# 959AI994/Multi-Gate-VAE

Measured on AMD Instinct MI355X. Metric: circuit-graphs/sec (train step), AIG-64k batch=64 per GPU, higher is better.
Workload: dtype f32 storage; dense products as bf16x3 split-precision MFMA, fp32 accumulate; 1 GPU; cfg2: DG_AE --type aig, 64 x 65536-node synthetic levelised DAGs per GPU (N=4194304, E=6558720, 120 levels), H=64, 4+4 rounds, layernorm, weights [1,4,4], negatives sampled; step includes the 7-scalar metrics copy (pinned, read one step behind); global_batch=64, parallelism=dp1

## Files before the change

### include/mgvae_hip.h

```cpp
#ifndef MGVAE_HIP_H
#define MGVAE_HIP_H
#include <stdint.h>
#ifdef __cplusplus
extern "C" {
#endif

#ifndef MGV_OK
#define MGV_OK 0
#define MGV_EINVAL (-1)
#define MGV_EUNSUPPORTED (-2)
#endif

int mgv_abi_version(void);

int mgv_struct_stage_fwd(int H, int64_t N, const float* h_in, const int32_t* nbr_ptr, const int32_t* nbr_idx,
                         const uint8_t* xcls, const float* xtab, int C, const float* Wc, const float* bc,
                         const float* Whh, const float* bhh, const float* ln_w, const float* ln_b, float ln_eps,
                         float* h_out, void* stream);
int mgv_struct_stage_bwd(int H, int64_t N, const float* h_in, const int32_t* nbr_ptr, const int32_t* nbr_idx,
                         const uint8_t* xcls, const float* xtab, int C, const float* Wc, const float* WcT,
                         const float* bc, const float* Whh, const float* WhhT, const float* bhh,
                         const float* ln_w, const float* ln_b, float ln_eps, const float* gy_direct,
                         const float* gy_agg, float* g_direct_out, float* g_agg_out, float* dWc, float* dbc,
                         float* dWhh, float* dbhh, float* dxtab, float* dln_w, float* dln_b, void* stream);
int mgv_struct_stage_rows_fwd(int H, int64_t N, const float* h_in, const int32_t* nbr_ptr, const int32_t* nbr_idx,
                              const float* xrow, const float* Wc, const float* bc, const float* Whh, const float* bhh,
                              const float* ln_w, const float* ln_b, float ln_eps, float* h_out, void* stream);
int mgv_struct_stage_rows_bwd(int H, int64_t N, const float* h_in, const int32_t* nbr_ptr, const int32_t* nbr_idx,
                              const float* xrow, const float* Wc, const float* WcT, const float* bc, const float* Whh,
                              const float* WhhT, const float* bhh, const float* ln_w, const float* ln_b, float ln_eps,
                              const float* gy_direct, const float* gy_agg, float* g_direct_out, float* g_agg_out,
                              float* dWc, float* dbc, float* dWhh, float* dbhh, float* d_xrow, float* dln_w, float* dln_b,
                              void* stream);

int mgv_struct_stage_fwd_x3(int H, int64_t N, const float* h_in, const int32_t* nbr_ptr, const int32_t* nbr_idx,
                            const uint8_t* xcls, const float* xtab, int C, const void* wpack_bf16, const float* bc,
                            const float* bhh, const float* ln_w, const float* ln_b, float ln_eps, float* h_out,
                            int heavy_n, const int32_t* heavy_nodes, float* heavy_ws, const int32_t* table_own_idx,
                            int nbr_tagged, float* ln_stats_out, void* stream);
int mgv_struct_stage_bwd_x3(int H, int64_t N, const float* h_in, const int32_t* nbr_ptr, const int32_t* nbr_idx,
                            const uint8_t* xcls, const float* xtab, int C, const void* wpack_bf16, const float* bc,
                            const float* bhh, const float* ln_w, const float* ln_b, float ln_eps,
                            const float* gy_direct, const float* gy_agg, float* g_direct_out, float* g_agg_out,
                            float* dWc, float* dbc, float* dWhh, float* dbhh, float* dxtab, float* dln_w,
                            float* dln_b, int heavy_n, const int32_t* heavy_nodes, float* heavy_ws, const int32_t* table_own_idx,
                            int nbr_tagged, void* stream);

int mgv_struct_stage_bwd2_ws_floats(int H, int64_t N);
int mgv_struct_stage_bwd2_x3(int H, int64_t N, const float* h_in, const int32_t* nbr_ptr, const int32_t* nbr_idx,
                             const uint8_t* xcls, const float* xtab, int C, const void* wpack_bf16, const float* bc,
                             const float* bhh, const float* ln_w, const float* ln_b, float ln_eps,
                             const float* gy_direct, const float* gy_agg, float* g_direct_out, float* g_agg_out,
                             float* dWc, float* dbc, float* dWhh, float* dbhh, float* dxtab, float* dln_w,
                             float* dln_b, float* workspace, int64_t workspace_floats, int heavy_n,
                             const int32_t* heavy_nodes, float* heavy_ws, const int32_t* table_own_idx,
                             int nbr_tagged, const float* ln_stats, void* stream);

int mgv_linear_fwd(int64_t N, const float* X1, int K1, int ld1, const float* X2, int K2, int ld2,
                   const float* W, const float* b, int M, float* Y, int ldy, void* stream);
int mgv_linear_wgrad(int64_t N, const float* X1, int K1, int ld1, const float* X2, int K2, int ld2,
                     const float* dY, int lddy, int M, float* dW, float* db, void* stream);
int mgv_linear_x3_supported(int M, int K);
int mgv_wpack_bf16x3(const float* W, int R, int K, int ldw, int transpose, void* hi, void* lo, void* stream);
int mgv_linear_fwd_x3(int64_t N, const float* X1, int K1, int ld1, const float* X2, int K2, int ld2,
                      const void* wpack_bf16, const float* b, int M, float* Y, int ldy, void* stream);
int mgv_grouped_linear_supported(int M, int K);
int mgv_grouped_linear_fwd_x3(int64_t ntiles, const int32_t* tile_list, const int32_t* order, const int32_t* tile_start,
                              const int32_t* tile_count, const int32_t* tile_slot, const float* X, int K, int ldx,
                              const void* wpack_bf16, const float* b, int M, const float* R, int ldr, float* Y, int ldy, void* stream);
int mgv_grouped_linear_wgrad_x3_ws_floats(int M, int K, int64_t ntiles);
int mgv_grouped_linear_wgrad_x3(int64_t ntiles, const int32_t* tile_list, const int32_t* order, const int32_t* tile_start,
                                const int32_t* tile_count, const float* X, int K, int ldx, const float* dY, int lddy, int M,
                                float* dW, float* db, float* workspace, int64_t workspace_floats, void* stream);
int mgv_linear_fwd_x3_res(int64_t N, const float* X1, int K1, int ld1, const float* X2, int K2, int ld2,
                          const void* wpack_bf16, const float* b, int M, const float* R, int ldr, float* Y, int ldy,
                          void* stream);
int mgv_linear_wgrad_x3_ws_floats(int M, int K, int64_t N);
int mgv_linear_wgrad_x3(int64_t N, const float* X1, int K1, int ld1, const float* X2, int K2, int ld2,
                        const float* dY, int lddy, int M, float* dW, float* db, float* workspace, int64_t workspace_floats,
                        void* stream);
int mgv_linear_bwd_x3_supported(int M, int K);
int mgv_linear_bwd_x3(int64_t N, const float* X1, int K1, int ld1, const float* X2, int K2, int ld2, const float* dY, int lddy,
                      int M, const void* wtpack_bf16, float* dW, float* db, float* dX1, int ldx1, float* dX2, int ldx2,
                      const float* R, int ldr, float* workspace, int64_t workspace_floats, void* stream);
int mgv_gather_sum(int H, int64_t N, const float* h, const int32_t* nbr_ptr, const int32_t* nbr_idx,
                   float* agg, float* deg, void* stream);

int mgv_class_expand(int H, int64_t N, const float* table, const int32_t* class_id, float* out, void* stream);
int mgv_seg_sum(int H, int64_t n_seg, const int32_t* seg_ptr, const int32_t* items, const float* direct, const float* agg,
// ... 276 lines not shown
```

### multi-gate-vae_amd/deepgate/_model_base.py

```python
import os

import torch
from torch import nn

from . import metrics, ops, pairs, similarity
from .arch.mlp import MLP
from .arch.tfmlp import TFMlpAggr
from .data import plan_of
from .digae_layer import DirectedInnerProductDecoder
from .sampling import NegativeEdges, negative_sampling, negative_sampling_device

EPS = 1e-15
DEVICE_SAMPLER = True
MAX_LOGSTD = 10


class FunctionalModel(nn.Module):
    ENCODER_ATTR = 'struct_encoder'
    GATES = ()

    VAR_HEADS = ('fc_s_mu', 'fc_s_logstd', 'fc_t_mu', 'fc_t_logstd')

    def __init__(self, struct_encoder, num_rounds=1, dim_hidden=128, enable_encode=True, enable_reverse=True, variational=False):
        super().__init__()
        setattr(self, self.ENCODER_ATTR, struct_encoder)
        self.decoder = DirectedInnerProductDecoder()
        self.hs_linear = nn.Linear(dim_hidden * 2, dim_hidden)
        self.hs_decompose = nn.Linear(dim_hidden, dim_hidden * 2)
        self.num_rounds = num_rounds
        self.enable_encode = enable_encode
        self.enable_reverse = enable_reverse
        self.dim_hidden = dim_hidden
        self.dim_mlp = 32
        for name, _ in self.GATES:
            setattr(self, 'aggr_%s_func' % name, TFMlpAggr(dim_hidden * 2, dim_hidden))
        for name, _ in self.GATES:
            setattr(self, 'update_%s_func' % name, nn.GRU(dim_hidden, dim_hidden))
        self.readout_prob = MLP(dim_hidden, self.dim_mlp, 1, num_layer=3, p_drop=0.2, norm_layer='batchnorm',
                                act_layer='relu')
        self.variational = bool(variational)
        if self.variational:
            for name in self.VAR_HEADS:
                setattr(self, name, nn.Linear(dim_hidden, dim_hidden))
        self._klsum, self._kl_n = None, 0
        self.last_confusion = None
        self.last_link_metrics = None
        self._neg_scope, self._neg_reverse = 'batch', 0.0

    def _sweep_params(self):
        parts = [getattr(self, 'aggr_%s_func' % n).composed(getattr(self, 'update_%s_func' % n)) for n, _ in self.GATES]
        return [torch.stack([p[i] for p in parts]) for i in range(5)]

    def forward(self, G, branch=None):
        if self.num_rounds < 1:
            raise ValueError('num_rounds must be >= 1')
        plan = plan_of(G, [gid for _, gid in self.GATES])
        dev = self.hs_linear.weight.device
        rows = torch.eye(6, dtype=torch.float32, device=dev)
        enc = getattr(self, self.ENCODER_ATTR)
        s, t = enc(None, None, G.edge_index, plan=plan, classes=(rows, plan.xcls))
        hs = ops.linear(s, self.hs_linear.weight, self.hs_linear.bias, x2=t)
        hs_in = hs
        if branch is not None:
            with branch.fork(hs):
                hs_in = branch.took(*self.recon_loss(hs, plan=plan, return_hs=True, **branch.recon_args))
        hf = ops.FuncSweepFn.apply(plan, hs_in, *self._sweep_params())
        if branch is not None:
            hf = branch.sweep_out(hf)
        for _ in range(self.num_rounds - 1):
            au, Wvc, bvc, bih, _ = self._sweep_params()
            hf = ops.FuncSweepFn.apply(plan, hs_in, au, Wvc, bvc, bih, None, hf, self._round_gh(plan, hf))
        return hs, hf

    def _round_gh(self, plan, hf):
        H = self.dim_hidden
        if hf.is_cuda and H == 64 and ops.use_x3(H) and ops.GROUPED_ROUND:
            grus = [getattr(self, 'update_%s_func' % name) for name, _ in self.GATES]
            return ops.RoundGhFn.apply(plan, hf, torch.stack([g.weight_hh_l0 for g in grus]), torch.stack([g.bias_hh_l0 for g in grus]))
        gh = torch.zeros(hf.shape[0], 3 * H, dtype=hf.dtype, device=hf.device)
        for (name, _), idx in zip(self.GATES, plan.slot_nodes()):
            if idx.numel() == 0:
                continue
            gru = getattr(self, 'update_%s_func' % name)
# ... 191 lines not shown
```

### multi-gate-vae_amd/deepgate/digae_layer.py

```python
import torch
import torch.nn as nn

from . import metrics, ops, pairs
from .arch.gcn_conv import AggConv
from .graph_plan import GraphPlan

MAX_FEATURE_CLASSES = 8


def feature_classes(x):
    rows, inv = torch.unique(x, dim=0, return_inverse=True)
    if rows.shape[0] > MAX_FEATURE_CLASSES:
        return None
    return rows.to(torch.float32), inv.to(torch.uint8).contiguous()


class DirectedInnerProductDecoder(nn.Module):

    def forward(self, s, t, edge_index, sigmoid=True):
        return ops.edge_dot(s, t, edge_index, sigmoid)

    def forward_all(self, s, t, sigmoid=True):
        return pairs.pair_scores(s, t, sigmoid)

# ... 110 lines not shown
    def forward(self, s_0, t_0, edge_index, plan=None, classes=None):
        if plan is None:
            plan = GraphPlan(edge_index, (classes[1] if classes is not None else s_0).shape[0])
        F_ = self.source_conv.conv.lin.in_features
        cs = _classes_once(s_0, classes, F_)
        ct = cs if (classes is not None or t_0 is s_0) else _classes_once(t_0, None, F_)
        return self.source_conv(t_0, edge_index, plan, ct), self.target_conv(s_0, edge_index, plan, cs)


class MultiGCNEncoder(nn.Module):
    def __init__(self, num_rounds, dim_hidden, dim_feature, enable_reverse, layernorm):
        super().__init__()
        self.num_rounds = num_rounds
        self.enable_reverse = True
        self.layernorm = layernorm
        self.dim_feature = dim_feature
        self.dim_hidden = dim_hidden
        self.aggr = AggConv(dim_hidden, dim_hidden)
        self.update = nn.GRU(dim_hidden + dim_feature, dim_hidden)
        self.aggr_r = AggConv(dim_hidden, dim_hidden)
        self.update_r = nn.GRU(dim_hidden + dim_feature, dim_hidden)
        if self.layernorm:
            self.ln = nn.LayerNorm(dim_hidden)

    def _composed(self, aggr, gru, feat_rows):
        H = self.dim_hidden
        w_ih = gru.weight_ih_l0
        w_m = w_ih[:, :H]
        Wc = w_m @ aggr.msg.weight
        bc = w_m @ aggr.msg.bias
        xtab = feat_rows @ w_ih[:, H:].t() + gru.bias_ih_l0
        return xtab, Wc, bc, gru.weight_hh_l0, gru.bias_hh_l0

    def _forward_rows(self, x, edge_index, plan):
        H, F_ = self.dim_hidden, self.dim_feature
        if plan is None:
            plan = GraphPlan(edge_index, x.shape[0])
        pad = (-F_) % 16
        xp = torch.nn.functional.pad(x.to(torch.float32), (0, pad)).contiguous()
        args = []
        for aggr, gru in ((self.aggr, self.update), (self.aggr_r, self.update_r)):
            w_ih = gru.weight_ih_l0
            w_m = w_ih[:, :H]
            w_x = torch.nn.functional.pad(w_ih[:, H:], (0, pad))
            xrow = torch.cat([ops.linear(xp, w_x[g * H:(g + 1) * H], gru.bias_ih_l0[g * H:(g + 1) * H]) for g in range(3)], dim=1)
            args += [xrow, w_m @ aggr.msg.weight, w_m @ aggr.msg.bias, gru.weight_hh_l0, gru.bias_hh_l0]
        ln_w = self.ln.weight if self.layernorm else None
        ln_b = self.ln.bias if self.layernorm else None
        return ops.StructEncoderRowsFn.apply(plan, self.num_rounds, *args, ln_w, ln_b)

    def forward(self, x, edge_index, plan=None, classes=None):
        if classes is None:
            if x.shape[1] != self.dim_feature:
                raise ValueError('expected %d node features, got %d' % (self.dim_feature, x.shape[1]))
            classes = feature_classes(x)
        if classes is None:
            return self._forward_rows(x, edge_index, plan)
        rows, xcls = classes
        if rows.shape[1] != self.dim_feature:
            raise ValueError('expected %d node features, got %d' % (self.dim_feature, rows.shape[1]))
        if plan is None:
            plan = GraphPlan(edge_index, xcls.shape[0])
        rows = rows.to(self.update.weight_ih_l0.device)
        f = self._composed(self.aggr, self.update, rows)
        r = self._composed(self.aggr_r, self.update_r, rows)
        ln_w = self.ln.weight if self.layernorm else None
        ln_b = self.ln.bias if self.layernorm else None
        return ops.StructEncoderFn.apply(plan, xcls, self.num_rounds, *f, *r, ln_w, ln_b)


class DirectMultiGCNEncoder(nn.Module):
    def __init__(self, dim_feature=3, dim_hidden=128, s_rounds=1, t_rounds=1, enable_reverse=True, layernorm=False):
        super().__init__()
        self.source_conv = MultiGCNEncoder(s_rounds, dim_hidden, dim_feature, enable_reverse, layernorm)
        self.target_conv = MultiGCNEncoder(t_rounds, dim_hidden, dim_feature, enable_reverse, layernorm)

    def forward(self, s, t, edge_index, plan=None, classes=None):
        if plan is None:
            plan = GraphPlan(edge_index, s.shape[0])
        cs = classes if classes is not None else feature_classes(s)
        ct = cs if (classes is not None or t is s) else feature_classes(t)
        return self.source_conv(s, edge_index, plan, cs), self.target_conv(t, edge_index, plan, ct)
```

### multi-gate-vae_amd/deepgate/ops.py

```python
from collections import namedtuple
import math
import os

import torch

from . import _hip
from ._hip import F32, I32, U8, HipLibraryError, check, edge_rows, ptr

LN_EPS = 1e-5

PRECISION = os.environ.get('MGV_PRECISION', 'x3')
FIRST_STAGE_TABLE = True


def use_x3(H):
    return PRECISION == 'x3' and H in (32, 64)


def split_bf16(w):
    hi = w.to(torch.bfloat16)
    lo = (w - hi.to(torch.float32)).to(torch.bfloat16)
    return hi, lo


# ... 7 lines not shown
    n = W.numel()
    if W.dtype != F32 or not W.is_cuda or W.stride(1) != 1:
        raise HipLibraryError('weight must be an fp32 GPU matrix with contiguous rows')
    base = out.data_ptr() + 2 * off
    _hip.call('mgv_wpack_bf16x3', ptr(W), R, K, W.stride(0), int(transpose), _hip.ctypes.c_void_p(base),
              _hip.ctypes.c_void_p(base + 2 * n))
    return off + 2 * n


def stage_wpack(Wc, Whh):
    out = torch.empty(4 * (Wc.numel() + Whh.numel()), dtype=torch.bfloat16, device=Wc.device)
    off = 0
    for w, tr in ((Wc, False), (Whh, False), (Wc, True), (Whh, True)):
        off = _pack_into(out, off, w, tr)
    return out


def sweep_wpack(Wvc):
    out = torch.empty(4 * Wvc.numel(), dtype=torch.bfloat16, device=Wvc.device)
    off = 0
    for g in range(Wvc.shape[0]):
        off = _pack_into(out, off, Wvc[g], False)
        off = _pack_into(out, off, Wvc[g], True)
    return out


def linear_wpack(W):
    out = torch.empty(2 * W.numel(), dtype=torch.bfloat16, device=W.device)
    _pack_into(out, 0, W, False)
    return out


def _zeros_like_params(*ts):
    return [torch.zeros_like(t) for t in ts]


def _heavy_args(heavy, H, device):
    if heavy is None or heavy[0] == 0:
        return 0, None, None
    n, nodes = heavy
    return n, ptr(nodes), ptr(workspace(2 * n * H, device, tag='heavy'))


def struct_stage_fwd(h_in, nbr_ptr, nbr_idx, xcls, xtab, Wc, bc, Whh, bhh, ln_w, ln_b, out=None, wpack=None, heavy=None, table_own=None, n_rows=None,
                     stats_out=None, tagged=True):
    N, H = h_in.shape
    if n_rows is not None:
        N = int(n_rows)
    if table_own is not None:
        N = table_own.numel()
    check(h_in, F32, 'h_in'); check(nbr_ptr, I32, 'nbr_ptr'); check(nbr_idx, I32, 'nbr_idx'); check(xcls, U8, 'xcls')
    for n, t in (('xtab', xtab), ('Wc', Wc), ('bc', bc), ('Whh', Whh), ('bhh', bhh)):
        check(t, F32, n)
    check(ln_w, F32, 'ln_w'); check(ln_b, F32, 'ln_b')
    assert nbr_ptr.numel() == N + 1 and xcls.numel() == N
    assert Wc.shape == (3 * H, H) and Whh.shape == (3 * H, H) and xtab.shape[1] == 3 * H
    h_out = (torch.empty(N, H, dtype=F32, device=h_in.device) if out is None else out)
    if use_x3(H):
        wpack = stage_wpack(Wc, Whh) if wpack is None else wpack
        _hip.call('mgv_struct_stage_fwd_x3', H, N, ptr(h_in), ptr(nbr_ptr), ptr(nbr_idx), ptr(xcls), ptr(xtab),
                  xtab.shape[0], ptr(wpack), ptr(bc), ptr(bhh), ptr(ln_w), ptr(ln_b), LN_EPS, ptr(h_out), *_heavy_args(heavy, H, h_in.device), ptr(table_own),
                  int(bool(tagged)), ptr(stats_out))
        return h_out
    assert table_own is None, 'table mode needs the bf16x3 kernels'
    _hip.call('mgv_struct_stage_fwd', H, N, ptr(h_in), ptr(nbr_ptr), ptr(nbr_idx), ptr(xcls), ptr(xtab),
              xtab.shape[0], ptr(Wc), ptr(bc), ptr(Whh), ptr(bhh), ptr(ln_w), ptr(ln_b), LN_EPS, ptr(h_out))
    return h_out
# ... 80 lines not shown


def half_round_schedule(plan, xcls, rounds, H, x3, first, quot):
    N, quot = plan.N, list(quot or [])[:2 * rounds]
    q = len(quot)
    table_mode = not q and first is not None and x3 and H == 64 and plan.tagged_fits(first[1])
    out = []
    for k in range(2 * rounds):
        rev = k % 2 == 1
        p, i = plan.csr(rev)
        if k < q:
            st = quot[k]
            if k + 1 < q:
                grad, gsrc = 'above', tuple(quot[k + 1][f] for f in ('own_levels', 'own_rows', 'ent_levels', 'ent_rows'))
            else:
                grad, gsrc = 'sum_levels', (st.get('sum_levels'), p, i)
            lists = (dict(idx=st['ent_idx'], table_own=st['own32'], tagged=False) if x3 else
                     dict(idx=st['idx'], n_rows=st['C'], src='stacked', own=st['own']))
            out.append(HalfRound(rev, st['C'], st['ptr'], xcls=st['xcls'], heavy=st['heavy'], expand=st['cid'] if k + 1 == q else None,
                                 grad=grad, gsrc=gsrc, **lists))
        elif k == 0 and first is not None:
            cid, C, tp, ti, tx = first
            out.append(HalfRound(rev, C, tp, ti, tx, None, src='ones', expand=None if table_mode else cid, grad='pairs', gsrc=(cid, p, i)))
        elif k == 1 and table_mode:
            out.append(HalfRound(rev, N, p, plan.tagged_idx(rev, first[0]), xcls, plan.heavy(rev), table_own=first[0]))
        else:
            out.append(HalfRound(rev, N, p, i, xcls, plan.heavy(rev), src='ones' if k == 0 else 'prev'))
    return out


class StructEncoderFn(torch.autograd.Function):

    @staticmethod
    def forward(ctx, plan, xcls, rounds, xtab_f, Wc_f, bc_f, Whh_f, bhh_f, xtab_r, Wc_r, bc_r, Whh_r, bhh_r, ln_w, ln_b):
        N = plan.N
        H = Whh_f.shape[1]
        dev = Whh_f.device
        par = [t.detach().contiguous() for t in (xtab_f, Wc_f, bc_f, Whh_f, bhh_f, xtab_r, Wc_r, bc_r, Whh_r, bhh_r)]
        lw = ln_w.detach().contiguous() if ln_w is not None else None
        lb = ln_b.detach().contiguous() if ln_b is not None else None
        packs = (stage_wpack(par[1], par[3]), stage_wpack(par[6], par[8])) if use_x3(H) else (None, None)
        quot = plan.quotient(xcls, 2 * rounds) if (QUOTIENT and FIRST_STAGE_TABLE and rounds > 0 and N > 0 and Whh_f.is_cuda) else []
        first = plan.first_stage_classes(xcls) if (not quot and FIRST_STAGE_TABLE and rounds > 0 and N > 0) else None
        sched = half_round_schedule(plan, xcls, rounds, H, use_x3(H), first, quot)
        keep_stats = lw is not None and use_x3(H) and H == 64
        states, stats = [], []
        h = torch.ones(1, H, dtype=F32, device=dev) if quot else None
        for r in sched:
            if r.src == 'ones':
                h = torch.ones(r.rows, H, dtype=F32, device=dev)
            elif r.src == 'stacked':
                h = torch.cat([h.index_select(0, r.own), h])
            states.append(None if r.grad == 'pairs' else h)
            stats.append(torch.empty(r.rows, 2, dtype=F32, device=dev) if keep_stats else None)
            h = struct_stage_fwd(h, r.ptr, r.idx, r.xcls, *(par[5:] if r.rev else par[:5]), lw, lb, wpack=packs[int(r.rev)], heavy=r.heavy,
                                 table_own=r.table_own, n_rows=r.n_rows, stats_out=stats[-1], tagged=r.tagged)
            if r.expand is not None:
                table, h = h, torch.empty(N, H, dtype=F32, device=dev)
                _hip.call('mgv_class_expand', H, N, ptr(table), ptr(r.expand), ptr(h))
        if not sched:
            h = torch.ones(N, H, dtype=F32, device=dev)
        ctx.plan, ctx.packs, ctx.sched = plan, packs, sched
        ctx.par, ctx.lw, ctx.lb, ctx.states, ctx.stats = par, lw, lb, states, stats
        return h

    @staticmethod
    def backward(ctx, gy):
        plan, par, lw, lb = ctx.plan, ctx.par, ctx.lw, ctx.lb
        H, dev = gy.shape[1], gy.device
        dlw = torch.zeros_like(lw) if lw is not None else None
        dlb = torch.zeros_like(lb) if lb is not None else None
        acc = [dict(zip(('dxtab', 'dWc', 'dbc', 'dWhh', 'dbhh', 'dln_w', 'dln_b'), _zeros_like_params(*w) + [dlw, dlb])) for w in (par[:5], par[5:])]
        g_direct, g_agg = gy.contiguous(), None
        for k in range(len(ctx.sched) - 1, -1, -1):
            r, h_in = ctx.sched[k], ctx.states[k]
            if r.grad == 'pairs':
                cid, p, i = r.gsrc
                gsum = torch.zeros(r.rows, H, dtype=F32, device=dev)
                ws = workspace(_hip.call_value('mgv_class_pull_sum_ws_floats', H, plan.N, r.rows), dev)
                _hip.call('mgv_class_pull_sum', H, plan.N, ptr(g_direct), ptr(g_agg), ptr(p), ptr(i), ptr(cid), r.rows, ptr(gsum), ptr(ws), ws.numel())
                g_direct, g_agg, h_in = gsum, None, torch.ones(r.rows, H, dtype=F32, device=dev)
            elif r.grad == 'sum_levels':
                (order, levels), p, i = r.gsrc
                flat = plan.seg_entries(r.rev, order, levels) if (SEG_LISTS and g_agg is not None) else None
                g_direct, g_agg = _seg_sums(H, levels, order, g_direct, g_agg, p, i, entries=flat), None
            elif r.grad == 'above':
                own_levels, own_rows, ent_levels, ent_rows = r.gsrc
                g_direct, g_agg = _seg_sums(H, own_levels, own_rows, g_direct) + _seg_sums(H, ent_levels, ent_rows, g_agg), None
            g_direct, g_agg = struct_stage_bwd(h_in, r.ptr, r.idx, r.xcls, *(par[5:] if r.rev else par[:5]), lw, lb, g_direct, g_agg, acc[int(r.rev)],
                                               need_input_grad=(k > 0), wpack=ctx.packs[int(r.rev)], heavy=r.heavy, table_own=r.table_own,
                                               n_rows=r.n_rows, stats=ctx.stats[k], tagged=r.tagged)
        ctx.states = ctx.stats = None
        f, r = acc
        return (None, None, None, f['dxtab'], f['dWc'], f['dbc'], f['dWhh'], f['dbhh'],
                r['dxtab'], r['dWc'], r['dbc'], r['dWhh'], r['dbhh'], dlw, dlb)


class StructEncoderRowsFn(torch.autograd.Function):

    @staticmethod
    def forward(ctx, plan, rounds, xrow_f, Wc_f, bc_f, Whh_f, bhh_f, xrow_r, Wc_r, bc_r, Whh_r, bhh_r, ln_w, ln_b):
        N, H, dev = plan.N, Whh_f.shape[1], Whh_f.device
        par = [check(t.detach().contiguous(), F32, 'encoder parameter') for t in (xrow_f, Wc_f, bc_f, Whh_f, bhh_f, xrow_r, Wc_r, bc_r, Whh_r, bhh_r)]
        lw = ln_w.detach().contiguous() if ln_w is not None else None
        lb = ln_b.detach().contiguous() if ln_b is not None else None
        assert par[0].shape == (N, 3 * H) and par[5].shape == (N, 3 * H)
        h = torch.ones(N, H, dtype=F32, device=dev)
        states = []
        for _ in range(rounds):
            for rev in (False, True):
                p, i = plan.csr(rev)
                w = par[5:] if rev else par[:5]
                states.append(h)
                out = torch.empty(N, H, dtype=F32, device=dev)
                _hip.call('mgv_struct_stage_rows_fwd', H, N, ptr(h), ptr(p), ptr(i), ptr(w[0]), ptr(w[1]), ptr(w[2]), ptr(w[3]), ptr(w[4]),
                          ptr(lw), ptr(lb), LN_EPS, ptr(out))
                h = out
        ctx.plan, ctx.rounds, ctx.par, ctx.lw, ctx.lb, ctx.states = plan, rounds, par, lw, lb, states
        return h

    @staticmethod
    def backward(ctx, gy):
        plan, par, lw, lb = ctx.plan, ctx.par, ctx.lw, ctx.lb
        N, H, dev = plan.N, gy.shape[1], gy.device
        acc = {}
        for tag, w in (('f', par[:5]), ('r', par[5:])):
            acc[tag] = [torch.zeros_like(t) for t in w]
            acc[tag] += [w[1].t().contiguous(), w[3].t().contiguous()]
# ... 338 lines not shown
        kp = (i32a * len(hav['lvl_k_ptr']))(*hav['lvl_k_ptr'])
        sp_ = (i32a * len(hav['lvl_seg_ptr']))(*hav['lvl_seg_ptr'])
        hws = workspace((hav['K'] + hav['S']) * 2 * H, dev, tag='heavy_active')
        ha = (hav['K'], ptr(hav['nodes']), ptr(hav['node_seg_ptr']), ptr(hav['seg_e0']), ptr(hav['seg_e1']), kp, sp_, ptr(hws), plan.HEAVY_ROW)
    return scratch, stp, hv, ha


SWEEP_X3_MAX_SLOTS = 6


def _sweep_x3(H, T=1):
    return use_x3(H) and T <= SWEEP_X3_MAX_SLOTS and os.environ.get('MGV_SWEEP_X3', '1') != '0'


GROUPED_ROUND = True

PACKED_ROWS = {'0': 0, '2': 2}.get(os.environ.get('MGV_PACKED_ROWS', '1'), 1)


def _sweep_rows(plan, forward=False):
    if PACKED_ROWS and forward and plan.__dict__.get('_order_rows') is None:
        steps = plan.__dict__.get('_sweep_steps', 0)
        plan._sweep_steps = steps + 1
        if PACKED_ROWS == 2 or steps >= 1:
            plan.order_rows
    if PACKED_ROWS and plan.__dict__.get('_order_rows') is not None:
        return ptr(plan.order_rows), 32
    return ptr(plan.order_span), 4


class FuncSweepFn(torch.autograd.Function):

    @staticmethod
    def forward(ctx, plan, hs, attn_u, Wvc, bvc, bih, bhh, hprev=None, gh=None):
        hsd = check(hs.detach().contiguous(), F32, 'hs')
        N, H = hsd.shape
        T = attn_u.shape[0]
        if bhh is None:
            bhh = torch.zeros(T, 3 * H, dtype=F32, device=hsd.device)
        par = [check(t.detach().contiguous(), F32, 'sweep parameter') for t in (attn_u, Wvc, bvc, bih, bhh)]
        assert plan.has_levels and plan.num_slots == T and plan.N == N
        hp = ghd = None
        if hprev is not None:
            hp = check(hprev.detach().contiguous(), F32, 'h_prev')
            ghd = check(gh.detach().contiguous(), F32, 'gh')
            assert ghd.shape == (N, 3 * H) and hp.shape == (N, H)
        ltp = (_hip.ctypes.c_int32 * len(plan.level_tile_ptr))(*plan.level_tile_ptr)
        wpack = sweep_wpack(par[1]) if _sweep_x3(H, T) else None
        if hp is not None:
            hf = hp.clone()
        elif wpack is not None:
            hf = torch.empty(N, H, dtype=F32, device=hsd.device)
            _hip.call('mgv_sweep_zero_inactive', H, N, ptr(plan.gslot), ptr(hf))
        else:
            hf = torch.zeros(N, H, dtype=F32, device=hsd.device)
        if wpack is not None:
            _hip.call('mgv_func_sweep_fwd_x3', H, N, T, plan.num_levels, ltp, ptr(plan.order), *_sweep_rows(plan, True),
                      ptr(plan.tile_start), ptr(plan.tile_count), ptr(plan.tile_slot), ptr(plan.in_ptr), ptr(plan.in_src), ptr(hsd), ptr(hf),
                      ptr(par[0]), ptr(wpack), ptr(par[2]), ptr(par[3]), ptr(par[4]), ptr(ghd), ptr(hp))
        else:
            _hip.call('mgv_func_sweep_fwd', H, N, T, plan.num_levels, ltp, ptr(plan.order), ptr(plan.tile_start),
                      ptr(plan.tile_count), ptr(plan.tile_slot), ptr(plan.in_ptr), ptr(plan.in_src), ptr(hsd), ptr(hf),
                      *[ptr(t) for t in par], ptr(ghd), ptr(hp))
        ctx.plan, ctx.par, ctx.ltp, ctx.wpack = plan, par, ltp, wpack
        ctx.save_for_backward(hsd, hf, hp, ghd)
        return hf

    @staticmethod
    def backward(ctx, ghf):
        plan, par = ctx.plan, ctx.par
        hs, hf, hp, ghd = ctx.saved_tensors
        N, H = hs.shape
        T = par[0].shape[0]
        dev = hs.device
        ghf = check(ghf.contiguous(), F32, 'ghf')
        ghs = (torch.empty if ctx.wpack is not None else torch.zeros)(N, H, dtype=F32, device=dev)
        dzb = torch.empty(N, 2 * H, dtype=F32, device=dev)
        alpha = torch.empty(max(plan.E, 1), dtype=F32, device=dev)
        dsc = torch.empty(max(plan.E, 1), dtype=F32, device=dev)
        grads = [torch.zeros_like(t) for t in par]
        d_gh = g_hprev = None
        if hp is not None:
            d_gh = torch.zeros(N, 3 * H, dtype=F32, device=dev)
            g_hprev = torch.zeros(N, H, dtype=F32, device=dev)
        rnd = (ptr(ghd), ptr(hp), ptr(d_gh), ptr(g_hprev))
        if ctx.wpack is not None:
            scratch, stp, hv, ha = _sweep_bwd_prep(plan, T, H, dev)
            _hip.call('mgv_func_sweep_bwd_x3', H, N, T, plan.num_levels, ctx.ltp, ptr(plan.order), *_sweep_rows(plan),
                      plan.n_active, ptr(plan.tile_start), ptr(plan.tile_count), ptr(plan.tile_slot), ptr(plan.slot_tiles), stp,
                      ptr(plan.in_ptr), ptr(plan.in_src), ptr(plan.out_ptr), ptr(plan.out_dst), ptr(plan.out_slot),
                      ptr(plan.gslot), ptr(hs), ptr(hf), ptr(par[0]), ptr(ctx.wpack), ptr(par[2]), ptr(par[3]), ptr(par[4]),
                      ptr(ghf), ptr(ghs), ptr(dzb), ptr(alpha), ptr(dsc), *[ptr(g) for g in grads], ptr(scratch),
                      scratch.numel(), plan.HEAVY_ROW if hv is not None else 0, *ha, *rnd)
            if hv is not None:
                pw = workspace(hv['S'] * H, dev)
                _hip.call('mgv_sweep_pull_heavy', H, hv['K'], ptr(hv['nodes']), ptr(hv['node_seg_ptr']), hv['S'], ptr(hv['seg_e0']), ptr(hv['seg_e1']),
                          ptr(plan.out_dst), ptr(plan.out_slot), ptr(plan.gslot), ptr(alpha), ptr(dsc), ptr(dzb), ptr(par[0]), ptr(pw), ptr(ghs))
        else:
            WvcT = par[1].transpose(1, 2).contiguous()
            _hip.call('mgv_func_sweep_bwd', H, N, T, plan.num_levels, ctx.ltp, ptr(plan.order), ptr(plan.tile_start),
                      ptr(plan.tile_count), ptr(plan.tile_slot), ptr(plan.in_ptr), ptr(plan.in_src), ptr(plan.out_ptr),
                      ptr(plan.out_dst), ptr(plan.out_slot), ptr(plan.gslot), ptr(hs), ptr(hf), ptr(par[0]), ptr(par[1]),
                      ptr(WvcT), ptr(par[2]), ptr(par[3]), ptr(par[4]), ptr(ghf), ptr(ghs), ptr(dzb), ptr(alpha), ptr(dsc),
                      *[ptr(g) for g in grads], *rnd)
        return (None, ghs, *grads[:4], grads[4] if hp is None else None, g_hprev, d_gh)


class EdgeDotFn(torch.autograd.Function):
    @staticmethod
    def forward(ctx, s, t, edge_index, sigmoid):
        sd, td = check(s.detach().contiguous(), F32, 's'), check(t.detach().contiguous(), F32, 't')
        src, dst = edge_rows(edge_index)
        E, H = src.numel(), sd.shape[1]
        out = torch.empty(E, dtype=F32, device=sd.device)
        _hip.call('mgv_edge_dot_fwd', H, E, ptr(sd), ptr(td), H, ptr(src), ptr(dst), int(bool(sigmoid)), ptr(out))
        ctx.save_for_backward(sd, td, src, dst)
        ctx.sigmoid = bool(sigmoid)
        return out

    @staticmethod
    def backward(ctx, gout):
        sd, td, src, dst = ctx.saved_tensors
        H = sd.shape[1]
        ds, dt = torch.zeros_like(sd), torch.zeros_like(td)
        gout = gout.contiguous()
        _hip.call('mgv_edge_dot_bwd', H, src.numel(), ptr(sd), ptr(td), H, ptr(src), ptr(dst), int(ctx.sigmoid),
                  ptr(gout), ptr(ds), ptr(dt))
        return ds, dt, None, None


def edge_dot(s, t, edge_index, sigmoid=True):
    return EdgeDotFn.apply(s, t, edge_index, sigmoid)


def _recon_heavy(plan):
    heavy = [(0, plan.heavy_segments(True), plan.out_dst), (1, plan.heavy_segments(False), plan.in_src)]
    return heavy, (plan.HEAVY_ROW if any(hv is not None for _, hv, _ in heavy) else 0)

# ... 436 lines not shown
```

Before: 1013 graphs/s.

## Fuse encoder and sweep weight composition and bf16 packing into native HIP kernels

Adds HIP kernels that build the composed struct-encoder and sweep weights, and pack them into bf16x3 hi/lo fragments in both orientations in one launch. Matching backward kernels replace the chains of small autograd matmuls. Parameter-gradient zero buffers are carved from a single allocation instead of many `zeros_like` calls. With the default setting the forward products are still computed in torch and the kernel only packs them. The sweep path is taken only when `num_rounds == 1`. The aim is to cut many tiny per-step launches and allocations, at the cost of more code paths and naive per-thread dot loops.

```diff
diff --git a/include/mgvae_hip.h b/include/mgvae_hip.h
--- a/include/mgvae_hip.h
+++ b/include/mgvae_hip.h
@@ -55,6 +55,14 @@
                              float* dln_b, float* workspace, int64_t workspace_floats, int heavy_n,
                              const int32_t* heavy_nodes, float* heavy_ws, const int32_t* table_own_idx,
                              int nbr_tagged, const float* ln_stats, void* stream);
+
+int mgv_struct_compose_fwd(int H, int n_dir, int C, int F, const float* rows, const float* const* in, float* const* out, int given,
+                           void* stream);
+int mgv_struct_compose_bwd(int H, int n_dir, int C, int F, const float* rows, const float* const* in, float* const* out, void* stream);
+int mgv_sweep_compose_fwd(int H, int T, const float* const* in, float* attn_u, float* Wvc, float* bvc, float* bih, float* bhh,
+                          void* wpack_bf16, int given, void* stream);
+int mgv_sweep_compose_bwd(int H, int T, const float* const* in, const float* dattn_u, const float* dWvc, const float* dbvc,
+                          float* const* out, void* stream);
 
 int mgv_linear_fwd(int64_t N, const float* X1, int K1, int ld1, const float* X2, int K2, int ld2,
                    const float* W, const float* b, int M, float* Y, int ldy, void* stream);
diff --git a/multi-gate-vae_amd/csrc/compose.hip b/multi-gate-vae_amd/csrc/compose.hip
--- /dev/null
+++ b/multi-gate-vae_amd/csrc/compose.hip
@@ -0,0 +1,240 @@
+#include "mgv_launch.h"
+#include "mgv_x3.h"
+#include "../../include/mgvae_hip.h"
+
+namespace mgv {
+
+constexpr int kComposeDirs = 4;
+constexpr int kComposeSlots = 6;
+
+__device__ __forceinline__ int frag_off(int row, int k, int K) {
+    const int blk = (row >> 4) * (K >> 5) + (k >> 5);
+    return (blk << 9) + (((((k & 31) >> 3) << 4) + (row & 15)) << 3) + (k & 7);
+}
+
+__device__ __forceinline__ void pack_both(__bf16* p, int tr, float v, int row, int k, int R, int K) {
+    __bf16 h, l;
+    split_bf16(v, h, l);
+    const int n = R * K, o = frag_off(row, k, K), ot = frag_off(k, row, R);
+    p[o] = h; p[n + o] = l;
+    p[tr + ot] = h; p[tr + n + ot] = l;
+}
+
+__device__ __forceinline__ float dot_chain(const float* a, int sa, const float* b, int sb, int n, float acc = 0.f) {
+    for (int k = 0; k < n; ++k) acc = fmaf(a[(int64_t)k * sa], b[(int64_t)k * sb], acc);
+    return acc;
+}
+
+struct StructDirFwd { const float *W_ih, *b_ih, *Wm, *bm, *Whh; float *Wc, *bc, *xtab; __bf16* pack; };
+struct StructFwdArgs { StructDirFwd d[kComposeDirs]; const float* rows; int C, F, given; };
+
+template <int H>
+__global__ __launch_bounds__(256) void k_struct_compose_fwd(StructFwdArgs a) {
+    constexpr int M = 3 * H, MH = M * H;
+    const StructDirFwd& d = a.d[blockIdx.y];
+    const int ld = H + a.F;
+    int t = blockIdx.x * 256 + threadIdx.x;
+    if (t < MH) {
+        const int i = t / H, j = t % H;
+        float v;
+        if (a.given) v = d.Wc[t];
+        else d.Wc[t] = v = dot_chain(d.W_ih + (int64_t)i * ld, 1, d.Wm + j, H, H);
+        pack_both(d.pack, 4 * MH, v, i, j, M, H);
+        return;
+    }
+    t -= MH;
+    if (t < MH) {
+        pack_both(d.pack + 2 * MH, 4 * MH, d.Whh[t], t / H, t % H, M, H);
+        return;
+    }
+    t -= MH;
+    if (a.given) return;
+    if (t < M) {
+        d.bc[t] = dot_chain(d.W_ih + (int64_t)t * ld, 1, d.bm, 1, H);
+        return;
+    }
+    t -= M;
+    if (t < a.C * M) {
+        const int c = t / M, i = t % M;
+        d.xtab[t] = dot_chain(a.rows + (int64_t)c * a.F, 1, d.W_ih + (int64_t)i * ld + H, 1, a.F) + d.b_ih[i];
+    }
+}
+
+struct StructDirBwd { const float *W_ih, *Wm, *bm, *dWc, *dbc, *dxtab; float *dW_ih, *db_ih, *dWm, *dbm; };
+struct StructBwdArgs { StructDirBwd d[kComposeDirs]; const float* rows; int C, F; };
+
+template <int H>
+__global__ __launch_bounds__(256) void k_struct_compose_bwd(StructBwdArgs a) {
+    constexpr int M = 3 * H;
+    const StructDirBwd& d = a.d[blockIdx.y];
+    const int ld = H + a.F;
+    int t = blockIdx.x * 256 + threadIdx.x;
+    if (t < M * ld) {
+        const int i = t / ld, k = t % ld;
+        d.dW_ih[t] = k < H ? fmaf(d.dbc[i], d.bm[k], dot_chain(d.dWc + (int64_t)i * H, 1, d.Wm + (int64_t)k * H, 1, H))
+                           : dot_chain(d.dxtab + i, M, a.rows + (k - H), a.F, a.C);
+        return;
+    }
+    t -= M * ld;
+    if (t < M) {
+        float acc = 0.f;
+        for (int c = 0; c < a.C; ++c) acc += d.dxtab[(int64_t)c * M + t];
+        d.db_ih[t] = acc;
+        return;
+    }
+    t -= M;
+    if (t < H * H) {
+        const int k = t / H, j = t % H;
+        d.dWm[t] = dot_chain(d.W_ih + k, ld, d.dWc + j, H, M);
+        return;
+    }
+    t -= H * H;
+    if (t < H) d.dbm[t] = dot_chain(d.W_ih + t, ld, d.dbc, 1, M);
+}
+
+struct SweepSlotFwd { const float *wa, *Wk, *Wv, *bv, *W_ih, *b_ih, *b_hh; };
+struct SweepFwdArgs { SweepSlotFwd s[kComposeSlots]; float *attn_u, *Wvc, *bvc, *bih, *bhh; __bf16* pack; int given; };
+
+template <int H>
+__global__ __launch_bounds__(256) void k_sweep_compose_fwd(SweepFwdArgs a) {
+    constexpr int M = 3 * H, K = 2 * H, MK = M * K;
+    const int slot = blockIdx.y;
+    const SweepSlotFwd& s = a.s[slot];
+    int t = blockIdx.x * 256 + threadIdx.x;
+    if (t < MK) {
+        const int i = t / K, k = t % K;
+        float v;
+        if (a.given) v = a.Wvc[(int64_t)slot * MK + t];
+        else a.Wvc[(int64_t)slot * MK + t] = v = dot_chain(s.W_ih + (int64_t)i * H, 1, s.Wv + k, K, H);
+        pack_both(a.pack + (int64_t)slot * 4 * MK, 2 * MK, v, i, k, M, K);
+        return;
+    }
+    if (a.given) return;
+    t -= MK;
+    if (t < K) {
+        a.attn_u[slot * K + t] = dot_chain(s.wa + H, 1, s.Wk + t, K, H);
+        return;
+    }
+    t -= K;
+    if (t < M) {
+        a.bvc[slot * M + t] = dot_chain(s.W_ih + (int64_t)t * H, 1, s.bv, 1, H);
+        a.bih[slot * M + t] = s.b_ih[t];
+        a.bhh[slot * M + t] = s.b_hh[t];
+    }
+}
+
+struct SweepSlotBwd { const float *wa, *Wk, *Wv, *bv, *W_ih; float *dwa, *dWk, *dWv, *dbv, *dW_ih; };
+struct SweepBwdArgs { SweepSlotBwd s[kComposeSlots]; const float *dattn_u, *dWvc, *dbvc; };
+
+template <int H>
+__global__ __launch_bounds__(256) void k_sweep_compose_bwd(SweepBwdArgs a) {
+    constexpr int M = 3 * H, K = 2 * H, MK = M * K;
+    const int slot = blockIdx.y;
+    const SweepSlotBwd& s = a.s[slot];
+    const float* du = a.dattn_u + slot * K;
+    const float* dW = a.dWvc + (int64_t)slot * MK;
+    const float* db = a.dbvc + slot * M;
+    int t = blockIdx.x * 256 + threadIdx.x;
+    if (t < M * H) {
+        const int i = t / H, o = t % H;
+        s.dW_ih[t] = fmaf(db[i], s.bv[o], dot_chain(dW + (int64_t)i * K, 1, s.Wv + (int64_t)o * K, 1, K));
+        return;
+    }
+    t -= M * H;
+    if (t < H * K) {
+        const int o = t / K, k = t % K;
+        s.dWv[t] = dot_chain(s.W_ih + o, H, dW + k, K, M);
+        s.dWk[t] = s.wa[H + o] * du[k];
+        return;
+    }
+    t -= H * K;
+    if (t < H) {
+        s.dbv[t] = dot_chain(s.W_ih + t, H, db, 1, M);
+        s.dwa[t] = 0.f;
+        s.dwa[H + t] = dot_chain(du, 1, s.Wk + (int64_t)t * K, 1, K);
+    }
+}
+
+inline bool all_set(const void* const* p, int n) {
+    if (!p) return false;
+    for (int i = 0; i < n; ++i)
+        if (!p[i]) return false;
+    return true;
+}
+
+}
+
+extern "C" int mgv_struct_compose_fwd(int H, int n_dir, int C, int F, const float* rows, const float* const* in, float* const* out,
+                                      int given, void* stream) {
+    if (!mgv::has_width(mgv::X3Widths{}, H)) return MGV_EUNSUPPORTED;
+    MGV_CHECK_ARG(n_dir >= 1 && n_dir <= mgv::kComposeDirs && C >= 1 && F >= 1 && rows);
+    MGV_CHECK_ARG(mgv::all_set(reinterpret_cast<const void* const*>(in), 5 * n_dir) && mgv::all_set(reinterpret_cast<const void* const*>(out), 4 * n_dir));
+    mgv::StructFwdArgs a{};
+    for (int d = 0; d < n_dir; ++d) {
+        const float* const* i = in + 5 * d;
+        float* const* o = out + 4 * d;
+        a.d[d] = {i[0], i[1], i[2], i[3], i[4], o[0], o[1], o[2], reinterpret_cast<__bf16*>(o[3])};
+    }
+    a.rows = rows; a.C = C; a.F = F; a.given = given != 0;
+    const int M = 3 * H, total = given ? 2 * M * H : 2 * M * H + M + C * M;
+    return mgv::launch_width(mgv::X3Widths{}, H, [&](auto w) {
+        hipLaunchKernelGGL((mgv::k_struct_compose_fwd<decltype(w)::value>), dim3((total + 255) / 256, n_dir), dim3(256), 0,
+                           static_cast<hipStream_t>(stream), a);
+    });
+}
+
+extern "C" int mgv_struct_compose_bwd(int H, int n_dir, int C, int F, const float* rows, const float* const* in, float* const* out,
+                                      void* stream) {
+    if (!mgv::has_width(mgv::X3Widths{}, H)) return MGV_EUNSUPPORTED;
+    MGV_CHECK_ARG(n_dir >= 1 && n_dir <= mgv::kComposeDirs && C >= 1 && F >= 1 && rows);
+    MGV_CHECK_ARG(mgv::all_set(reinterpret_cast<const void* const*>(in), 6 * n_dir) && mgv::all_set(reinterpret_cast<const void* const*>(out), 4 * n_dir));
+    mgv::StructBwdArgs a{};
+    for (int d = 0; d < n_dir; ++d) {
+        const float* const* i = in + 6 * d;
+        float* const* o = out + 4 * d;
+        a.d[d] = {i[0], i[1], i[2], i[3], i[4], i[5], o[0], o[1], o[2], o[3]};
+    }
+    a.rows = rows; a.C = C; a.F = F;
+    const int M = 3 * H, total = M * (H + F) + M + H * H + H;
+    return mgv::launch_width(mgv::X3Widths{}, H, [&](auto w) {
+        hipLaunchKernelGGL((mgv::k_struct_compose_bwd<decltype(w)::value>), dim3((total + 255) / 256, n_dir), dim3(256), 0,
+                           static_cast<hipStream_t>(stream), a);
+    });
+}
+
+extern "C" int mgv_sweep_compose_fwd(int H, int T, const float* const* in, float* attn_u, float* Wvc, float* bvc, float* bih, float* bhh,
+                                     void* wpack_bf16, int given, void* stream) {
+    if (!mgv::has_width(mgv::X3Widths{}, H)) return MGV_EUNSUPPORTED;
+    MGV_CHECK_ARG(T >= 1 && T <= mgv::kComposeSlots && attn_u && Wvc && bvc && bih && bhh && wpack_bf16);
+    MGV_CHECK_ARG(mgv::all_set(reinterpret_cast<const void* const*>(in), 7 * T));
+    mgv::SweepFwdArgs a{};
+    for (int s = 0; s < T; ++s) {
+        const float* const* i = in + 7 * s;
+        a.s[s] = {i[0], i[1], i[2], i[3], i[4], i[5], i[6]};
+    }
+    a.attn_u = attn_u; a.Wvc = Wvc; a.bvc = bvc; a.bih = bih; a.bhh = bhh; a.pack = static_cast<__bf16*>(wpack_bf16); a.given = given != 0;
+    const int total = given ? 6 * H * H : 6 * H * H + 2 * H + 3 * H;
+    return mgv::launch_width(mgv::X3Widths{}, H, [&](auto w) {
+        hipLaunchKernelGGL((mgv::k_sweep_compose_fwd<decltype(w)::value>), dim3((total + 255) / 256, T), dim3(256), 0,
+                           static_cast<hipStream_t>(stream), a);
+    });
+}
+
+extern "C" int mgv_sweep_compose_bwd(int H, int T, const float* const* in, const float* dattn_u, const float* dWvc, const float* dbvc,
+                                     float* const* out, void* stream) {
+    if (!mgv::has_width(mgv::X3Widths{}, H)) return MGV_EUNSUPPORTED;
+    MGV_CHECK_ARG(T >= 1 && T <= mgv::kComposeSlots && dattn_u && dWvc && dbvc);
+    MGV_CHECK_ARG(mgv::all_set(reinterpret_cast<const void* const*>(in), 5 * T) && mgv::all_set(reinterpret_cast<const void* const*>(out), 5 * T));
+    mgv::SweepBwdArgs a{};
+    for (int s = 0; s < T; ++s) {
+        const float* const* i = in + 5 * s;
+        float* const* o = out + 5 * s;
+        a.s[s] = {i[0], i[1], i[2], i[3], i[4], o[0], o[1], o[2], o[3], o[4]};
+    }
+    a.dattn_u = dattn_u; a.dWvc = dWvc; a.dbvc = dbvc;
+    const int total = 3 * H * H + 2 * H * H + H;
+    return mgv::launch_width(mgv::X3Widths{}, H, [&](auto w) {
+        hipLaunchKernelGGL((mgv::k_sweep_compose_bwd<decltype(w)::value>), dim3((total + 255) / 256, T), dim3(256), 0,
+                           static_cast<hipStream_t>(stream), a);
+    });
+}
diff --git a/multi-gate-vae_amd/deepgate/_model_base.py b/multi-gate-vae_amd/deepgate/_model_base.py
--- a/multi-gate-vae_amd/deepgate/_model_base.py
+++ b/multi-gate-vae_amd/deepgate/_model_base.py
@@ -48,7 +48,14 @@
         self._neg_scope, self._neg_reverse = 'batch', 0.0
 
     def _sweep_params(self):
-        parts = [getattr(self, 'aggr_%s_func' % n).composed(getattr(self, 'update_%s_func' % n)) for n, _ in self.GATES]
+        mods = [(getattr(self, 'aggr_%s_func' % n), getattr(self, 'update_%s_func' % n)) for n, _ in self.GATES]
+        if self.num_rounds == 1 and ops._sweep_x3(self.dim_hidden, len(mods)):
+            raw = [p for a, g in mods for p in (a.attn_lin.weight, a.msg_k.weight, a.msg_v.weight, a.msg_v.bias,
+                                                g.weight_ih_l0, g.bias_ih_l0, g.bias_hh_l0)]
+            if ops.compose_native(self.dim_hidden, *raw):
+                au, Wvc, bvc, bih, bhh, wpack = ops.SweepComposeFn.apply(*raw)
+                return [au, Wvc, bvc, bih, bhh, None, None, wpack]
+        parts = [a.composed(g) for a, g in mods]
         return [torch.stack([p[i] for p in parts]) for i in range(5)]
 
     def forward(self, G, branch=None):
diff --git a/multi-gate-vae_amd/deepgate/digae_layer.py b/multi-gate-vae_amd/deepgate/digae_layer.py
--- a/multi-gate-vae_amd/deepgate/digae_layer.py
+++ b/multi-gate-vae_amd/deepgate/digae_layer.py
@@ -166,6 +166,13 @@
         xtab = feat_rows @ w_ih[:, H:].t() + gru.bias_ih_l0
         return xtab, Wc, bc, gru.weight_hh_l0, gru.bias_hh_l0
 
+    def _raw(self):
+        return [p for aggr, gru in ((self.aggr, self.update), (self.aggr_r, self.update_r))
+                for p in (gru.weight_ih_l0, gru.bias_ih_l0, aggr.msg.weight, aggr.msg.bias, gru.weight_hh_l0)]
+
+    def compose_native(self, rows):
+        return rows.shape[1] == self.dim_feature and ops.compose_native(self.dim_hidden, *self._raw())
+
     def _forward_rows(self, x, edge_index, plan):
         H, F_ = self.dim_hidden, self.dim_feature
         if plan is None:
@@ -183,7 +190,7 @@
         ln_b = self.ln.bias if self.layernorm else None
         return ops.StructEncoderRowsFn.apply(plan, self.num_rounds, *args, ln_w, ln_b)
 
-    def forward(self, x, edge_index, plan=None, classes=None):
+    def forward(self, x, edge_index, plan=None, classes=None, composed=None):
         if classes is None:
             if x.shape[1] != self.dim_feature:
                 raise ValueError('expected %d node features, got %d' % (self.dim_feature, x.shape[1]))
@@ -196,10 +203,16 @@
         if plan is None:
             plan = GraphPlan(edge_index, xcls.shape[0])
         rows = rows.to(self.update.weight_ih_l0.device)
+        ln_w = self.ln.weight if self.layernorm else None
+        ln_b = self.ln.bias if self.layernorm else None
+        if composed is None and self.compose_native(rows):
+            composed = ops.StructComposeFn.apply(rows, *self._raw())
+        if composed is not None:
+            xf, Wf, bf, pf, xr, Wr, br, pr = composed
+            return ops.StructEncoderFn.apply(plan, xcls, self.num_rounds, xf, Wf, bf, self.update.weight_hh_l0, self.update.bias_hh_l0,
+                                             xr, Wr, br, self.update_r.weight_hh_l0, self.update_r.bias_hh_l0, ln_w, ln_b, pf, pr)
         f = self._composed(self.aggr, self.update, rows)
         r = self._composed(self.aggr_r, self.update_r, rows)
-        ln_w = self.ln.weight if self.layernorm else None
-        ln_b = self.ln.bias if self.layernorm else None
         return ops.StructEncoderFn.apply(plan, xcls, self.num_rounds, *f, *r, ln_w, ln_b)
 
 
@@ -214,4 +227,10 @@
             plan = GraphPlan(edge_index, s.shape[0])
         cs = classes if classes is not None else feature_classes(s)
         ct = cs if (classes is not None or t is s) else feature_classes(t)
-        return self.source_conv(s, edge_index, plan, cs), self.target_conv(t, edge_index, plan, ct)
+        src, tgt = self.source_conv, self.target_conv
+        if (cs is not None and ct is not None and cs[0] is ct[0] and src.dim_hidden == tgt.dim_hidden
+                and src.compose_native(cs[0]) and tgt.compose_native(cs[0])):
+            rows = cs[0].to(src.update.weight_ih_l0.device)
+            comp = ops.StructComposeFn.apply(rows, *src._raw(), *tgt._raw())
+            return src(s, edge_index, plan, cs, composed=comp[:8]), tgt(t, edge_index, plan, ct, composed=comp[8:])
+        return src(s, edge_index, plan, cs), tgt(t, edge_index, plan, ct)
diff --git a/multi-gate-vae_amd/deepgate/ops.py b/multi-gate-vae_amd/deepgate/ops.py
--- a/multi-gate-vae_amd/deepgate/ops.py
+++ b/multi-gate-vae_amd/deepgate/ops.py
@@ -63,7 +63,7 @@
 
 
 def _zeros_like_params(*ts):
-    return [torch.zeros_like(t) for t in ts]
+    return _carve(torch.zeros(sum(t.numel() for t in ts), dtype=ts[0].dtype, device=ts[0].device), [tuple(t.shape) for t in ts])
 
 
 def _heavy_args(heavy, H, device):
@@ -210,14 +210,19 @@
 class StructEncoderFn(torch.autograd.Function):
 
     @staticmethod
-    def forward(ctx, plan, xcls, rounds, xtab_f, Wc_f, bc_f, Whh_f, bhh_f, xtab_r, Wc_r, bc_r, Whh_r, bhh_r, ln_w, ln_b):
+    def forward(ctx, plan, xcls, rounds, xtab_f, Wc_f, bc_f, Whh_f, bhh_f, xtab_r, Wc_r, bc_r, Whh_r, bhh_r, ln_w, ln_b, pack_f=None, pack_r=None):
         N = plan.N
         H = Whh_f.shape[1]
         dev = Whh_f.device
         par = [t.detach().contiguous() for t in (xtab_f, Wc_f, bc_f, Whh_f, bhh_f, xtab_r, Wc_r, bc_r, Whh_r, bhh_r)]
         lw = ln_w.detach().contiguous() if ln_w is not None else None
         lb = ln_b.detach().contiguous() if ln_b is not None else None
-        packs = (stage_wpack(par[1], par[3]), stage_wpack(par[6], par[8])) if use_x3(H) else (None, None)
+        if not use_x3(H):
+            packs = (None, None)
+        elif pack_f is not None and pack_r is not None:
+            packs = (pack_f, pack_r)
+        else:
+            packs = (stage_wpack(par[1], par[3]), stage_wpack(par[6], par[8]))
         quot = plan.quotient(xcls, 2 * rounds) if (QUOTIENT and FIRST_STAGE_TABLE and rounds > 0 and N > 0 and Whh_f.is_cuda) else []
         first = plan.first_stage_classes(xcls) if (not quot and FIRST_STAGE_TABLE and rounds > 0 and N > 0) else None
         sched = half_round_schedule(plan, xcls, rounds, H, use_x3(H), first, quot)
@@ -246,9 +251,9 @@
     def backward(ctx, gy):
         plan, par, lw, lb = ctx.plan, ctx.par, ctx.lw, ctx.lb
         H, dev = gy.shape[1], gy.device
-        dlw = torch.zeros_like(lw) if lw is not None else None
-        dlb = torch.zeros_like(lb) if lb is not None else None
-        acc = [dict(zip(('dxtab', 'dWc', 'dbc', 'dWhh', 'dbhh', 'dln_w', 'dln_b'), _zeros_like_params(*w) + [dlw, dlb])) for w in (par[:5], par[5:])]
+        zeros = _zeros_like_params(*par, *((lw, lb) if lw is not None else ()))
+        dlw, dlb = zeros[10:] if lw is not None else (None, None)
+        acc = [dict(zip(('dxtab', 'dWc', 'dbc', 'dWhh', 'dbhh', 'dln_w', 'dln_b'), z + [dlw, dlb])) for z in (zeros[:5], zeros[5:10])]
         g_direct, g_agg = gy.contiguous(), None
         for k in range(len(ctx.sched) - 1, -1, -1):
             r, h_in = ctx.sched[k], ctx.states[k]
@@ -271,7 +276,7 @@
         ctx.states = ctx.stats = None
         f, r = acc
         return (None, None, None, f['dxtab'], f['dWc'], f['dbc'], f['dWhh'], f['dbhh'],
-                r['dxtab'], r['dWc'], r['dbc'], r['dWhh'], r['dbhh'], dlw, dlb)
+                r['dxtab'], r['dWc'], r['dbc'], r['dWhh'], r['dbhh'], dlw, dlb, None, None)
 
 
 class StructEncoderRowsFn(torch.autograd.Function):
@@ -676,7 +681,7 @@
 class FuncSweepFn(torch.autograd.Function):
 
     @staticmethod
-    def forward(ctx, plan, hs, attn_u, Wvc, bvc, bih, bhh, hprev=None, gh=None):
+    def forward(ctx, plan, hs, attn_u, Wvc, bvc, bih, bhh, hprev=None, gh=None, wpack=None):
         hsd = check(hs.detach().contiguous(), F32, 'hs')
         N, H = hsd.shape
         T = attn_u.shape[0]
@@ -690,7 +695,10 @@
             ghd = check(gh.detach().contiguous(), F32, 'gh')
             assert ghd.shape == (N, 3 * H) and hp.shape == (N, H)
         ltp = (_hip.ctypes.c_int32 * len(plan.level_tile_ptr))(*plan.level_tile_ptr)
-        wpack = sweep_wpack(par[1]) if _sweep_x3(H, T) else None
+        if not _sweep_x3(H, T):
+            wpack = None
+        elif wpack is None:
+            wpack = sweep_wpack(par[1])
         if hp is not None:
             hf = hp.clone()
         elif wpack is not None:
@@ -722,7 +730,7 @@
         dzb = torch.empty(N, 2 * H, dtype=F32, device=dev)
         alpha = torch.empty(max(plan.E, 1), dtype=F32, device=dev)
         dsc = torch.empty(max(plan.E, 1), dtype=F32, device=dev)
-        grads = [torch.zeros_like(t) for t in par]
+        grads = _zeros_like_params(*par)
         d_gh = g_hprev = None
         if hp is not None:
             d_gh = torch.zeros(N, 3 * H, dtype=F32, device=dev)
@@ -747,7 +755,115 @@
                       ptr(plan.out_dst), ptr(plan.out_slot), ptr(plan.gslot), ptr(hs), ptr(hf), ptr(par[0]), ptr(par[1]),
                       ptr(WvcT), ptr(par[2]), ptr(par[3]), ptr(par[4]), ptr(ghf), ptr(ghs), ptr(dzb), ptr(alpha), ptr(dsc),
                       *[ptr(g) for g in grads], *rnd)
-        return (None, ghs, *grads[:4], grads[4] if hp is None else None, g_hprev, d_gh)
+        return (None, ghs, *grads[:4], grads[4] if hp is None else None, g_hprev, d_gh, None)
+
+
+COMPOSE = os.environ.get('MGV_COMPOSE', 'hip')
+
+
+def compose_native(H, *params):
+    return COMPOSE != 'torch' and use_x3(H) and all(p.is_cuda and p.dtype == F32 and p.is_contiguous() for p in params)
+
+
+def _ptr_table(tensors):
+    return (_hip.ctypes.c_void_p * len(tensors))(*[t.data_ptr() for t in tensors])
+
+
+def _carve(buf, shapes):
+    out, off = [], 0
+    for shape in shapes:
+        n = math.prod(shape)
+        out.append(buf[off:off + n].view(shape))
+        off += n
+    assert off == buf.numel()
+    return out
+
+
+def _grad_or_zeros(g, shape, device):
+    return torch.zeros(shape, dtype=F32, device=device) if g is None else g.contiguous()
+
+
+class StructComposeFn(torch.autograd.Function):
+
+    @staticmethod
+    def forward(ctx, rows, *params):
+        n_dir = len(params) // 5
+        assert len(params) == 5 * n_dir and 1 <= n_dir <= 4
+        par = [check(p.detach(), F32, 'encoder parameter') for p in params]
+        rows = check(rows.detach().contiguous(), F32, 'rows')
+        H, (C, F_) = par[4].shape[1], rows.shape
+        M, dev = 3 * H, rows.device
+        for d in range(n_dir):
+            shapes = [tuple(t.shape) for t in par[5 * d:5 * d + 5]]
+            assert shapes == [(M, H + F_), (M,), (H, H), (H,), (M, H)], shapes
+        given = COMPOSE != 'native'
+        if given:
+            out = [t for d in range(n_dir) for w_ih, b_ih, wm, bm in (par[5 * d:5 * d + 4],)
+                   for t in (rows @ w_ih[:, H:].t() + b_ih, w_ih[:, :H] @ wm, w_ih[:, :H] @ bm)]
+        else:
+            out = _carve(torch.empty(n_dir * (C * M + M * H + M), dtype=F32, device=dev), [(C, M), (M, H), (M,)] * n_dir)
+        packs = torch.empty(n_dir, 8 * M * H, dtype=torch.bfloat16, device=dev)
+        table = [t for d in range(n_dir) for t in (check(out[3 * d + 1], F32, 'Wc'), out[3 * d + 2], out[3 * d], packs[d])]
+        _hip.call('mgv_struct_compose_fwd', H, n_dir, C, F_, ptr(rows), _ptr_table(par), _ptr_table(table), int(given))
+        ctx.par, ctx.rows, ctx.n_dir = par, rows, n_dir
+        res = tuple(t for d in range(n_dir) for t in (*out[3 * d:3 * d + 3], packs[d]))
+        ctx.mark_non_differentiable(*res[3::4])
+        ctx.set_materialize_grads(False)
+        return res
+
+    @staticmethod
+    def backward(ctx, *grads):
+        par, rows, n_dir = ctx.par, ctx.rows, ctx.n_dir
+        H, (C, F_) = par[4].shape[1], rows.shape
+        M = 3 * H
+        shapes = ((C, M), (M, H), (M,))
+        g = [check(_grad_or_zeros(grads[4 * d + i], shapes[i], rows.device), F32, 'gradient') for d in range(n_dir) for i in (1, 2, 0)]
+        ins = [t for d in range(n_dir) for t in (par[5 * d], par[5 * d + 2], par[5 * d + 3], *g[3 * d:3 * d + 3])]
+        out = _carve(torch.empty(n_dir * (M * (H + F_) + M + H * H + H), dtype=F32, device=rows.device), [(M, H + F_), (M,), (H, H), (H,)] * n_dir)
+        _hip.call('mgv_struct_compose_bwd', H, n_dir, C, F_, ptr(rows), _ptr_table(ins), _ptr_table(out))
+        return (None, *[t for d in range(n_dir) for t in (*out[4 * d:4 * d + 4], None)])
+
+
+class SweepComposeFn(torch.autograd.Function):
+
+    @staticmethod
+    def forward(ctx, *params):
+        T = len(params) // 7
+        assert len(params) == 7 * T and 1 <= T <= SWEEP_X3_MAX_SLOTS
+        par = [check(p.detach(), F32, 'sweep parameter') for p in params]
+        H = par[4].shape[1]
+        M, K, dev = 3 * H, 2 * H, par[0].device
+        for s_ in range(T):
+            shapes = [tuple(t.shape) for t in par[7 * s_:7 * s_ + 7]]
+            assert shapes == [(1, K), (H, K), (H, K), (H,), (M, H), (M,), (M,)], shapes
+        given = COMPOSE != 'native'
+        if given:
+            slots = [par[7 * s_:7 * s_ + 7] for s_ in range(T)]
+            au = torch.stack([wa[0, H:] @ wk for wa, wk, _, _, _, _, _ in slots])
+            Wvc = torch.stack([w_ih @ wv for _, _, wv, _, w_ih, _, _ in slots])
+            bvc = torch.stack([w_ih @ bv for _, _, _, bv, w_ih, _, _ in slots])
+            bih, bhh = torch.stack([p[5] for p in slots]), torch.stack([p[6] for p in slots])
+        else:
+            au, Wvc, bvc, bih, bhh = _carve(torch.empty(T * (K + M * K + 3 * M), dtype=F32, device=dev), [(T, K), (T, M, K), (T, M), (T, M), (T, M)])
+        wpack = torch.empty(T * 4 * M * K, dtype=torch.bfloat16, device=dev)
+        _hip.call('mgv_sweep_compose_fwd', H, T, _ptr_table(par), ptr(au), ptr(check(Wvc, F32, 'Wvc')), ptr(bvc), ptr(bih), ptr(bhh), ptr(wpack), int(given))
+        ctx.par, ctx.T = par, T
+        ctx.mark_non_differentiable(wpack)
+        ctx.set_materialize_grads(False)
+        return au, Wvc, bvc, bih, bhh, wpack
+
+    @staticmethod
+    def backward(ctx, dau, dWvc, dbvc, dbih, dbhh, _):
+        par, T = ctx.par, ctx.T
+        H = par[4].shape[1]
+        M, K = 3 * H, 2 * H
+        dev = par[0].device
+        dau, dWvc, dbvc, dbih, dbhh = (check(_grad_or_zeros(t, shape, dev), F32, 'gradient')
+                                       for t, shape in zip((dau, dWvc, dbvc, dbih, dbhh), ((T, K), (T, M, K), (T, M), (T, M), (T, M))))
+        ins = [t for s_ in range(T) for t in par[7 * s_:7 * s_ + 5]]
+        out = _carve(torch.empty(T * (K + 2 * H * K + H + M * H), dtype=F32, device=dev), [(1, K), (H, K), (H, K), (H,), (M, H)] * T)
+        _hip.call('mgv_sweep_compose_bwd', H, T, _ptr_table(ins), ptr(dau), ptr(dWvc), ptr(dbvc), _ptr_table(out))
+        return tuple(t for s_ in range(T) for t in (*out[5 * s_:5 * s_ + 5], dbih[s_], dbhh[s_]))
 
 
 class EdgeDotFn(torch.autograd.Function):
```

Result: no change. 1022 graphs/s (median of 6 runs) (+0.9%).
